# muhanzhang/IGMC

Measured on AMD Instinct MI355X. Metric: enclosing-subgraphs/sec (train step, batch=50) + test RMSE, higher is better.
Workload: dtype f32; 1 GPU; ml_1m, hop 1, max-nodes-per-hop 100, batch 50 per GPU, adj-dropout 0, dynamic-train, ARR 0.001, Adam; parallelism=dp1, global_batch=50, graphs_captured_before_timing=True, steps_per_graph_launch=100, group_steps=50

## Files before the change

igmc_amd/csrc/capi.hip:

```cpp
#include "launch.h"
#include "sortpool.h"
#include "g2_image.h"

#include <algorithm>
#include <climits>
#include <cmath>
#include <cstdio>
#include <cstring>
#include <map>
#include <string>
#include <vector>

static thread_local std::string g_err;
int g_igmc_prof_on = 0;

#define IGMC_FAIL(msg)                                                      \
  do {                                                                      \
    g_err = std::string(__func__) + ": " + (msg);                           \
    return 1;                                                               \
  } while (0)
#define HIPCHECK(expr)                                                      \
  do {                                                                      \
    hipError_t e_ = (expr);                                                 \
    if (e_ != hipSuccess) {                                                 \
// ... 652 lines not shown
    d.off_basis[l] = off; off += (int64_t)4 * fin * 32;
    d.off_root[l] = off;  off += (int64_t)fin * 32;
    d.off_bias[l] = off;  off += 32;
    d.off_att[l] = off;   off += (int64_t)d.R * 4;
  }
  d.off_l1w = off; off += (int64_t)128 * d.D;
  d.off_l1b = off; off += 128;
  d.off_l2w = off; off += 128;
  d.off_l2b = off; off += 1;
  d.n_params = off;
  d.node_cap = max_nodes;
  d.edge_cap = max_edges;
  d.graph_cap = max_graphs;
  Allocs& M = m->mem;
  int fail = 0;
  const size_t N = (size_t)max_nodes, Bc = (size_t)max_graphs;
  for (int l = 0; l < 4; ++l) fail |= M.get(&d.h[l], N * 32) | M.get(&d.dpre[l], N * 32);
  fail |= M.get(&d.agg, N * 128);
  for (int l = 0; l < 3; ++l) fail |= M.get(&d.gagg[l], N * 128) | M.get(&d.Y[l], N * 128);
  fail |= M.get(&d.feat, Bc * d.D) | M.get(&d.a1, Bc * 128) | M.get(&d.lmask, Bc * 128) | M.get(&d.dz, Bc * 128) |
          M.get(&d.gfeat, Bc * d.D) | M.get(&d.err, Bc) | M.get(&d.cnt0, N * d.R * d.L);
  const size_t rows0 = (size_t)d.R * d.L + d.L + 1;
  d.ts_part = nullptr;
  d.ts_raw = nullptr;
  d.ts_stride = (d.R * 32 + 33) * 32;
  d.fin_stash = nullptr;
  d.datt_part = nullptr;
  d.fold_w = nullptr;
  if (d.R <= G2_NR * G2_NG_MAX)
  {
    fail |= M.get(&d.ts_part, (size_t)4 * IGMC_TS_BLOCKS * d.ts_stride) |
            M.get(&d.ts_raw, (size_t)4 * d.ts_stride + (size_t)4 * d.ts_stride / 32 * 4);
    if (!fail) d.datt_part = d.ts_raw + (size_t)4 * d.ts_stride;
    fail |= M.get(&d.fold_w, (size_t)4 * 32 * IGMC_FOLD_NA);
  }
  if (d.R <= 128) fail |= M.get(&d.fin_stash, (size_t)4 * IGMC_STASH_LAYER + 16);
  d.g2_ex = nullptr;
  d.g2_fx = nullptr;
  d.g2_px = nullptr;
  d.g2_px_stride = 0;
  d.g2_w = nullptr;
  d.g2_graphs = 0;
  d.ex_nodes = 256;
  d.g2_ex_stride = (size_t)Bc * 2 * 32 * d.ex_nodes;
  const int wide = d.R <= G2_NR * G2_NG_MAX;
  const int xcd_ok = igmc_g2_xcd_ok();
  if (wide && Bc <= 2048 && xcd_ok) {
    fail |= M.get(&d.g2_ex, 5 * d.g2_ex_stride) | M.get(&d.g2_fx, Bc * 256) | M.get(&d.g2_w, g2_w_words(d.R, d.L));
    d.g2_graphs = (int)Bc;
    if (d.R <= G2_NR && Bc <= 1024) {
      d.g2_px_stride = (size_t)Bc * 2 * 32768;
      fail |= M.get(&d.g2_px, 5 * d.g2_px_stride);
    } else if (d.R <= G2_NR) {
      static bool told = false;
      if (!told) fprintf(stderr, "[igmc] batches of more than 1024 subgraphs: no plane-exchange regions -- the dense-layer / per-layer kernels take the steps, not the subgraph kernel\n");
      told = true;
    }
  } else if (wide) {
    fail |= M.get(&d.g2_w, g2_w_words(d.R, d.L));
  }
  fail |= M.get(&d.gs_bar, 2 * Bc + 1);
  fail |= M.get(&d.gs_ts, 4);
  d.gs_err = d.gs_bar ? d.gs_bar + 2 * Bc : nullptr;
  fail |= M.get(&d.wg_part, (size_t)4 * IGMC_WG_BLOCKS * igmc_wg_stride()) |
          M.get(&d.gatt_part, (size_t)3 * IGMC_GATHER_BLOCKS * d.R * 4) |
          M.get(&d.l0_part, (size_t)IGMC_L0_BLOCKS * rows0 * 32) |
          M.get(&d.graw, (size_t)3 * igmc_wg_stride() + 3 * d.R * 4 + rows0 * 32) | M.get(&d.arr_part, 4);
  d.side = nullptr;
  d.ctrl = nullptr;
  d.dcat[0] = d.dcat[1] = d.dcat[2] = nullptr;
  fail |= M.get(&m->done_ctr, 8);
  if (fail) {
    M.release();
    delete m;
    IGMC_FAIL("hipMalloc failed (model workspace)");
  }
  {
    hipStream_t st1, st2;
    if (hipStreamCreateWithFlags(&st1, hipStreamNonBlocking) != hipSuccess ||
        hipStreamCreateWithFlags(&st2, hipStreamNonBlocking) != hipSuccess) {
      M.release();
      delete m;
      IGMC_FAIL("hipStreamCreate failed");
    }
    m->ax.s1 = st1;
    m->ax.s2 = st2;
    for (int i = 0; i < 8; ++i) {
      hipEvent_t e;
      if (hipEventCreateWithFlags(&e, hipEventDisableTiming) != hipSuccess) IGMC_FAIL("hipEventCreate failed");
      m->ax.ev[i] = e;
    }
  }
  HIPCHECK(hipMemset(m->done_ctr, 0, 8 * sizeof(int)));
  HIPCHECK(hipMemset(m->d.gs_bar, 0, (2 * (size_t)max_graphs + 1) * sizeof(int)));
  {
    const unsigned long long ts0[4] = {~0ull, 0ull, 0ull, 0ull};
    HIPCHECK(hipMemcpy(m->d.gs_ts, ts0, sizeof(ts0), hipMemcpyHostToDevice));
  }
  if (m->d.fold_w) HIPCHECK(hipMemset(m->d.fold_w, 0, (size_t)4 * 32 * IGMC_FOLD_NA * sizeof(unsigned long long)));
  if (m->d.g2_ex) {
    HIPCHECK(hipMemset(m->d.g2_ex, 0, 5 * m->d.g2_ex_stride * sizeof(unsigned long long)));
    HIPCHECK(hipMemset(m->d.g2_fx, 0, (size_t)max_graphs * 256 * sizeof(unsigned long long)));
    if (m->d.g2_px) HIPCHECK(hipMemset(m->d.g2_px, 0, 5 * m->d.g2_px_stride));
  }
  if (igmc_model_prepare(d)) {
    M.release();
    delete m;
    IGMC_FAIL("hipFuncSetAttribute failed");
  }
  *out = m;
  return 0;
}

extern "C" int igmc_debug_lin_mask(const igmc_model* m, uint8_t* h_out, int64_t n) {
  if (!m || !h_out) IGMC_FAIL("null argument");
  if (n < 0 || n > (int64_t)m->d.graph_cap * 128) IGMC_FAIL("mask size out of range");
  HIPCHECK(hipDeviceSynchronize());
  HIPCHECK(hipMemcpy(h_out, m->d.lmask, (size_t)n, hipMemcpyDeviceToHost));
  return 0;
}

extern "C" int igmc_debug_head_array(const igmc_model* m, int which, float* h_out, int64_t n) {
  if (!m || !h_out) IGMC_FAIL("null argument");
  if (which < 0 || which > 3) IGMC_FAIL("no such array");
  const float* src = which == 0 ? m->d.a1 : which == 1 ? m->d.dz : which == 2 ? m->d.feat : m->d.gfeat;
  if (n < 0 || n > (int64_t)m->d.graph_cap * (which < 2 ? 128 : m->d.D)) IGMC_FAIL("size out of range");
  HIPCHECK(hipDeviceSynchronize());
  HIPCHECK(hipMemcpy(h_out, src, (size_t)n * sizeof(float), hipMemcpyDeviceToHost));
  return 0;
}

extern "C" int igmc_debug_weight_images(const igmc_model* m, float* h_out, int64_t* n_words) {
// ... 297 lines not shown

extern "C" int igmc_ctrl_tick(int64_t* d_ctrl, void* stream) {
  if (!d_ctrl) IGMC_FAIL("null ctrl");
  igmc_launch_tick(d_ctrl, stream);
  HIPCHECK(hipGetLastError());
  return 0;
}
extern "C" int igmc_ctrl_regroup(int64_t* d_ctrl, int M, int64_t first_cur, int64_t first_next, void* stream) {
  if (!d_ctrl || M < 1 || first_cur < 0 || first_next < 0) IGMC_FAIL("bad arguments");
  igmc_launch_regroup(d_ctrl, M, first_cur, first_next, stream);
  HIPCHECK(hipGetLastError());
  return 0;
}
extern "C" int igmc_ctrl_gate(int64_t* d_ctrl, int q, int gk_min, double delay_us, int delay_always, double timeout_us,
                              void* stream) {
  if (!d_ctrl || gk_min < 0 || !(timeout_us >= 0.0) || !(delay_us >= 0.0) || delay_us > 1000.0) IGMC_FAIL("bad arguments");
  igmc_launch_gate(d_ctrl, q & 1, gk_min, (long long)(delay_us * 100.0), delay_always != 0, (long long)(timeout_us * 100.0), stream);
  HIPCHECK(hipGetLastError());
  return 0;
}
extern "C" int igmc_batch_set_ctrl(igmc_batch* b, const int64_t* d_ctrl) {
  if (!b) IGMC_FAIL("null batch");
  b->ctrl = d_ctrl;
  return 0;
}
extern "C" int igmc_model_set_ctrl(igmc_model* m, const int64_t* d_ctrl) {
  if (!m) IGMC_FAIL("null model");
  m->d.ctrl = d_ctrl;
  return 0;
}
extern "C" int igmc_model_reset_exchange(igmc_model* m, void* stream) {
  if (!m) IGMC_FAIL("null model");
  hipStream_t st = (hipStream_t)stream;
  if (m->d.fold_w) HIPCHECK(hipMemsetAsync(m->d.fold_w, 0, (size_t)4 * 32 * IGMC_FOLD_NA * sizeof(unsigned long long), st));
  if (m->d.g2_ex) {
    HIPCHECK(hipMemsetAsync(m->d.g2_ex, 0, 5 * m->d.g2_ex_stride * sizeof(unsigned long long), st));
    HIPCHECK(hipMemsetAsync(m->d.g2_fx, 0, (size_t)m->d.g2_graphs * 256 * sizeof(unsigned long long), st));
    if (m->d.g2_px) HIPCHECK(hipMemsetAsync(m->d.g2_px, 0, 5 * m->d.g2_px_stride, st));
  }
  return 0;
}
extern "C" int igmc_model_check(igmc_model* m, void* stream) {
  if (!m) IGMC_FAIL("null model");
  int v = 0;
  if (m->d.gs_err) {
    HIPCHECK(hipStreamSynchronize((hipStream_t)stream));
    HIPCHECK(hipMemcpy(&v, m->d.gs_err, sizeof(int), hipMemcpyDeviceToHost));
    if (v) {
      HIPCHECK(hipMemset(m->d.gs_bar, 0, (2 * (size_t)m->d.graph_cap + 1) * sizeof(int)));
      (void)igmc_model_reset_exchange(m, stream);
      HIPCHECK(hipStreamSynchronize((hipStream_t)stream));
      IGMC_FAIL("a workgroup-cluster exchange of k_graph_step2 or a hand-off of the one-launch tail k_tail_fin timed out (GPU "
                "shared with another job?): results of the affected steps are invalid; set IGMC_GS_CLUSTER=1 or "
                "IGMC_GRAPH_STEP=0 (the tail alone: IGMC_TAIL_FOLD=0)");
    }
  }
  return 0;
}
extern "C" int igmc_adam_step_ctrl(float* d_params, const float* d_grad, float* d_exp_avg, float* d_exp_avg_sq,
                                   int64_t n, const int64_t* d_ctrl, void* stream) {
  if (!d_params || !d_grad || !d_exp_avg || !d_exp_avg_sq || n <= 0 || !d_ctrl) IGMC_FAIL("bad arguments");
  igmc_launch_adam(d_params, d_grad, d_exp_avg, d_exp_avg_sq, n, 0.f, 0.f, 0.f, 0.f, 0.f, 0.f, (int64_t*)d_ctrl, 0, stream);
  HIPCHECK(hipGetLastError());
  return 0;
}

extern "C" int igmc_step_finish(igmc_model* m, const igmc_batch* b, float* d_params, const float* d_grad,
// ... 604 lines not shown
```

igmc_amd/csrc/model.h:

```cpp
#pragma once
#include "common.h"

#define IGMC_KCAT 160
#ifndef IGMC_WG_BLOCKS
#define IGMC_WG_BLOCKS 64
#endif
#define IGMC_STASH_LAYER 672
#define IGMC_FOLD_NA 32
#define IGMC_TS_BLOCKS 256
#define IGMC_GATHER_BLOCKS 4096
#define IGMC_FBS_MAX_R 32
#define IGMC_L0_BLOCKS 256
#define IGMC_HG 8

struct ModelDev {
  int R, Bs, L, S, D;
  int64_t off_basis[4], off_root[4], off_bias[4], off_att[4];
  int64_t off_l1w, off_l1b, off_l2w, off_l2b, n_params;
  int node_cap, edge_cap, graph_cap;
  float* h[4];
  float* agg;
  float* gagg[3];
  float* Y[3];
  float* dpre[4];
  float* feat;
  float* a1;
  uint8_t* lmask;
  float* dz;
  float* gfeat;
  float* err;
  uint16_t* cnt0;
  float* wg_part;
  float* gatt_part;
  float* l0_part;
  float* graw;
  float* ts_part;
  float* ts_raw;
  int ts_stride;
  float* fin_stash;
  float* datt_part;
  unsigned long long* fold_w;
// ... 71 lines not shown
```

igmc_amd/csrc/model.hip:

```cpp
#include "model.h"
#include "g2_image.h"
#include "fin_stash.h"
#include "g2_words.h"
#include <stdlib.h>

struct XcdSeg {
  int lo, hi;
  int j, nj;
};
__device__ __forceinline__ XcdSeg igmc_xcd_segment(const BatchDev& b) {
  XcdSeg s;
  const int B = b.totals[3];
  const int x = blockIdx.x & 7;
  s.j = blockIdx.x >> 3;
  s.nj = (gridDim.x + 7 - x) >> 3;
  s.lo = b.node_off[(x * B) >> 3];
  s.hi = b.node_off[((x + 1) * B) >> 3];
  return s;
}


template <bool FLAGS, bool STORE>
__global__ __launch_bounds__(IGMC_BLOCK) void k_l0_fwd(BatchDev b, ModelDev m, const float* __restrict__ P,
                                                         float* __restrict__ out) {
  igmc_kernarg_warm<sizeof(BatchDev) + sizeof(ModelDev) + 32>();
  IGMC_DYN_SMEM(smem);
  const int RL = m.R * m.L, LF = m.L * 32;
  float* sW0 = (float*)smem;
  float* sroot = sW0 + RL * 32;
  float* sbias = sroot + LF;
  int* shist = (int*)(sbias + 32);
  for (int i = threadIdx.x; i < RL * 32; i += IGMC_BLOCK) {
    const int r = i / LF, cf = i % LF;
    float s = 0.f;
#pragma unroll
    for (int bb = 0; bb < 4; ++bb) s += P[m.off_att[0] + r * 4 + bb] * P[m.off_basis[0] + bb * LF + cf];
    sW0[i] = s;
// ... 1835 lines not shown
        const float anew = fts_att_entry(grad, at, st, R, rb, g, arr_coef, i, pold, m1o, m2o, part == 0);
        if (emit) s_attn[rb] = anew;
       }
      }
    }
    if (has) {
      if (table) {
        fts_col_table8(g, st, tv, R);
        for (int r = 8; r < R; ++r) {
          const float tvr = t0[(size_t)r * nE + e];
#pragma unroll
          for (int bb = 0; bb < 4; ++bb) g[bb] += st[IGMC_STASH_ATT + r * 4 + bb] * tvr;
        }
      }
      fts_col_emit(grad, at, st, arr_coef, idx, g, pv, m1v, m2v, pn);
      e_img = e;
    }
    if (emit) {
      __syncthreads();
      if (e_img >= 0) fts_image_col(m, ng, l, R, fin, e_img >> 5, e_img & 31, s_attn, pn, 0, 1);
    }
  } else if ((int)blockIdx.x < 4 * IGMC_FTS_NB + nlin) {
    const int64_t n_lin = m.n_params - m.off_l1w;
    const int64_t chunk = (n_lin + nlin - 1) / nlin;
    const int64_t lo = m.off_l1w + (int64_t)(blockIdx.x - 4 * IGMC_FTS_NB) * chunk;
    const int64_t hi = (lo + chunk < m.n_params) ? lo + chunk : m.n_params;
    adam_range<8>(at.p, grad, at.m1, at.m2, lo, hi, at.step_size, at.inv_sqrt_bc2, at.beta1, at.beta2, at.eps, at.wd);
  } else {
    loss_body(at.b, m, at.ARR, at.loss, at.total, smf);
    if (tid == 0 && at.ctrl) ctrl_check_and_advance(at.ctrl, at.b, at.use_flags);
  }
}

#define IGMC_TF_SETS 3
#define IGMC_TF_ROWS 384
#define IGMC_TF_O_ROWS (IGMC_TF_SETS * 1024)
#define IGMC_TF_O_ST (IGMC_TF_O_ROWS + IGMC_TF_ROWS)
#define IGMC_TF_O_DATT (IGMC_TF_O_ST + IGMC_STASH_LAYER)
#define IGMC_TF_O_ATTN (IGMC_TF_O_DATT + 32 * IGMC_FOLD_NA)
#define IGMC_TF_O_PN (IGMC_TF_O_ATTN + 64)
#define IGMC_TF_O_SMF (IGMC_TF_O_PN + 5 * 32)
#define IGMC_TF_WORDS (IGMC_TF_O_SMF + 16)
#define IGMC_TF_POLL ((32 * IGMC_FOLD_NA + IGMC_BLOCK - 1) / IGMC_BLOCK)
#define IGMC_TF_TIMEOUT_TICKS 20000000ll
#define IGMC_SYNC_ERR_FOLD 8

#if defined(IGMC_FIN_CLOCKS) && !defined(IGMC_HIPEMU)
__device__ unsigned long long g_fin_clk[64];
extern "C" int igmc_debug_fin_clocks(unsigned long long* out) {
  return hipMemcpyFromSymbol(out, HIP_SYMBOL(g_fin_clk), sizeof(g_fin_clk)) != hipSuccess;
}
#define TF_STAMP(on, k) do { if ((on) && threadIdx.x == 0) g_fin_clk[k] = __builtin_readcyclecounter(); } while (0)
#else
#define TF_STAMP(on, k) do { } while (0)
#endif

__global__ __launch_bounds__(IGMC_BLOCK) void k_tail_fin(BatchDev b, ModelDev m, const float* P, float grad_scale, float mult,
                                                           float drop_scale, float* grad, float arr_coef, AdamTail at, int nlin,
                                                           int nparts, int stride, int B, int bump_seq, int mute_layer) {
  __builtin_amdgcn_s_setprio(3);
  igmc_kernarg_warm<sizeof(BatchDev) + sizeof(ModelDev) + sizeof(AdamTail) + 64>();
  IGMC_DYN_SMEM(smem);
  float* S = (float*)smem;
  const int tid = threadIdx.x, lane = tid & 63, wave = tid >> 6;
  const float* stash = m.fin_stash;
  if (at.ctrl) {
    at.step_size = stash[IGMC_STASH_SCAL + 0];
    at.inv_sqrt_bc2 = stash[IGMC_STASH_SCAL + 1];
    at.beta1 = stash[IGMC_STASH_SCAL + 2];
    at.beta2 = stash[IGMC_STASH_SCAL + 3];
    at.eps = stash[IGMC_STASH_SCAL + 4];
    at.wd = stash[IGMC_STASH_SCAL + 5];
  }
  const int R = m.R, L = m.L, na = R * 4;
  const int nconv = 96 + L;
  const int blk = blockIdx.x;
  TF_STAMP(blk == 0, 0);
  TF_STAMP(blk == nconv, 16);
  TF_STAMP(blk == nconv + nlin, 32);
  if (blk < nconv) {
    const int l = blk < 96 ? 1 + (blk >> 5) : 0, c = blk < 96 ? (blk & 31) : blk - 96;
    const int fin = (l == 0) ? L : 32, nE = fin * 32, ts = m.ts_stride;
    const uint32_t tag = __float_as_uint(stash[IGMC_STASH_SCAL + IGMC_STASH_SEQ]) * 2u + 1u;
    float4* sred4 = (float4*)S;
    float* rows = S + IGMC_TF_O_ROWS;
    float* s_st = S + IGMC_TF_O_ST;
    float* s_datt = S + IGMC_TF_O_DATT;
    float* s_attn = S + IGMC_TF_O_ATTN;
    float* s_pn = S + IGMC_TF_O_PN;
    int* s_flag = (int*)(S + IGMC_TF_O_SMF + 8);
    const int ng = g2_groups(R, L);
    const int o4 = lane & 15, pg = wave * 4 + (lane >> 4);
    float stq[(IGMC_STASH_LAYER + IGMC_BLOCK - 1) / IGMC_BLOCK];
#pragma unroll
    for (int u = 0; u < (IGMC_STASH_LAYER + IGMC_BLOCK - 1) / IGMC_BLOCK; ++u) {
      const int i = tid + u * IGMC_BLOCK;
      stq[u] = stash[l * IGMC_STASH_LAYER + (i < IGMC_STASH_LAYER ? i : IGMC_STASH_LAYER - 1)];
    }
    const int f = tid & 31, e = c * 32 + f;
    const bool col = tid < 32, bias_role = c == 0 && tid >= 32 && tid < 64;
    int64_t idx[5];
    float pv[5], m1v[5], m2v[5], pvb[4] = {0.f, 0.f, 0.f, 0.f}, bq[4] = {0.f, 0.f, 0.f, 0.f};
#pragma unroll
    for (int q = 0; q < 5; ++q) {
      idx[q] = (q < 4) ? m.off_basis[l] + (int64_t)q * nE + e : m.off_root[l] + e;
      pv[q] = col ? P[idx[q]] : 0.f;
      m1v[q] = col ? at.m1[idx[q]] : 0.f;
      m2v[q] = col ? at.m2[idx[q]] : 0.f;
    }
    if (wave == 0) {
#pragma unroll
      for (int bb = 0; bb < 4; ++bb) pvb[bb] = P[idx[bb]];
    }
    if (bias_role) {
      const int64_t i = m.off_bias[l] + f;
      bq[1] = P[i];
      bq[2] = at.m1[i];
      bq[3] = at.m2[i];
    }
    if (tid == 0) *s_flag = 0;
    TF_STAMP(blk == 0, 1);
    const float* pl = m.ts_part + (size_t)l * IGMC_TS_BLOCKS * ts;
    const TsSlots sl = ts_slots(nparts, stride, B);
    const int nq = sl.nq;
    bool first_round = true;
    auto sum_columns = [&](int k0, int k1) {
      const int nsets = (k1 - k0 + 15) >> 4;
      int i0[IGMC_TF_SETS];
      float4 s4[IGMC_TF_SETS];
#pragma unroll
      for (int s = 0; s < IGMC_TF_SETS; ++s) {
        const int k = k0 + 16 * s + o4, kc = k < k1 ? k : k1 - 1, j = kc >> 3;
        const int row = j < R ? j * fin + c : j == R ? R * fin + c : R * fin + fin;
        i0[s] = row * 32 + 4 * (kc & 7);
        s4[s] = make_float4(0.f, 0.f, 0.f, 0.f);
      }
      for (int q0 = pg; q0 < nq; q0 += 16 * 14) {
        float4 v[IGMC_TF_SETS][14];
        size_t so[14];
#pragma unroll
        for (int u = 0; u < 14; ++u) so[u] = (size_t)ts_slot(sl, q0 + 16 * u) * ts;
#pragma unroll
        for (int s = 0; s < IGMC_TF_SETS; ++s)
          if (s < nsets) {
#pragma unroll
            for (int u = 0; u < 14; ++u) v[s][u] = *(const float4*)(pl + so[u] + i0[s]);
          }
#pragma unroll
        for (int s = 0; s < IGMC_TF_SETS; ++s)
          if (s < nsets) {
#pragma unroll
            for (int u = 0; u < 14; ++u)
              if (q0 + 16 * u < nq) {
                s4[s].x += v[s][u].x; s4[s].y += v[s][u].y; s4[s].z += v[s][u].z; s4[s].w += v[s][u].w;
              }
          }
      }
      if (!first_round) __syncthreads();
#pragma unroll
      for (int s = 0; s < IGMC_TF_SETS; ++s)
        if (s < nsets) sred4[(s * 16 + pg) * 16 + o4] = s4[s];
      if (first_round) {
#pragma unroll
        for (int u = 0; u < (IGMC_STASH_LAYER + IGMC_BLOCK - 1) / IGMC_BLOCK; ++u) {
          const int i = tid + u * IGMC_BLOCK;
          if (i < IGMC_STASH_LAYER) s_st[i] = stq[u];
        }
      }
      first_round = false;
      __syncthreads();
      if (wave < nsets) {
        const float* sr = (const float*)sred4;
        float tot = 0.f;
#pragma unroll
        for (int g16 = 0; g16 < 16; ++g16) tot += sr[((wave * 16 + g16) * 16 + (lane >> 2)) * 4 + (lane & 3)];
        const int k = k0 + 16 * wave + (lane >> 2);
        if (k < k1) rows[k * 4 + (lane & 3)] = tot;
      }
    };
    const int ncol_a = 8 * (R + 1);
    for (int k0 = 0; k0 < ncol_a; k0 += 16 * IGMC_TF_SETS) sum_columns(k0, k0 + 16 * IGMC_TF_SETS < ncol_a ? k0 + 16 * IGMC_TF_SETS : ncol_a);
    __syncthreads();
    TF_STAMP(blk == 0, 2);
    unsigned long long* words = m.fold_w + (size_t)l * 32 * IGMC_FOLD_NA;
    if (wave == 0) {
      const int h = lane >> 5;
      for (int r2 = 0; r2 < R; r2 += 2) {
        const int r = r2 + h;
        const float tot = r < R ? rows[r * 32 + f] : 0.f;
        float pb[4];
#pragma unroll
        for (int bb = 0; bb < 4; ++bb) pb[bb] = tot * pvb[bb];
#pragma unroll
        for (int bb = 0; bb < 4; ++bb)
#pragma unroll
          for (int d = 16; d >= 1; d >>= 1) pb[bb] += __shfl_xor(pb[bb], d, 64);
#ifdef IGMC_HIPEMU
        if (l == mute_layer) continue;
#endif
        if (f == 0 && r < R) {
#pragma unroll
          for (int bb = 0; bb < 4; ++bb) g2_pub_f32_agent(words + c * IGMC_FOLD_NA + r * 4 + bb, pb[bb], tag);
        }
      }
    }
    TF_STAMP(blk == 0, 3);
    if (c == 0) sum_columns(ncol_a, ncol_a + 8);
    TF_STAMP(blk == 0, 4);
    {
      const int nw = fin * na;
      const unsigned long long* wp[IGMC_TF_POLL];
      int wi[IGMC_TF_POLL];
#pragma unroll
      for (int u = 0; u < IGMC_TF_POLL; ++u) {
        const int w = tid + u * IGMC_BLOCK, wc = w < nw ? w : nw - 1;
        wi[u] = (wc / na) * IGMC_FOLD_NA + wc % na;
        wp[u] = words + wi[u];
      }
      bool ok = false;
#ifndef IGMC_HIPEMU
      const long long t0 = (long long)wall_clock64();
#endif
      for (long it = 0;; ++it) {
        unsigned long long w[IGMC_TF_POLL];
        bool all = true;
#pragma unroll
        for (int u = 0; u < IGMC_TF_POLL; ++u) w[u] = g2_ld_word(wp[u]);
#pragma unroll
        for (int u = 0; u < IGMC_TF_POLL; ++u) all = all && (uint32_t)(w[u] >> 32) == tag;
        if (all) {
#pragma unroll
          for (int u = 0; u < IGMC_TF_POLL; ++u) s_datt[wi[u]] = __uint_as_float((uint32_t)w[u]);
          ok = true;
          break;
        }
#ifndef IGMC_HIPEMU
        if ((it & 15) == 15 && (long long)wall_clock64() - t0 > IGMC_TF_TIMEOUT_TICKS) break;
        __builtin_amdgcn_s_sleep(2);
#else
        if (it > (1L << 12)) break;
        hipemu::yield();
#endif
      }
      if (!ok) *s_flag = 1;
    }
    __syncthreads();
    TF_STAMP(blk == 0, 5);
    if (*s_flag) {
      if (tid == 0) {
        *m.gs_err = 1;
        if (at.ctrl) atomicOr((unsigned long long*)(at.ctrl + IGMC_CTRL_SYNC_ERR), (unsigned long long)IGMC_SYNC_ERR_FOLD);
      }
      return;
    }
    const float* st = s_st;
    if (tid >= 64 && tid - 64 < na) {
      const int rb = tid - 64;
      float g = 0.f;
#pragma unroll
      for (int k = 0; k < 32; ++k) g += (k < fin) ? s_datt[k * IGMC_FOLD_NA + rb] : 0.f;
      s_attn[rb] = fts_att_entry(grad, at, st, R, rb, g, arr_coef, m.off_att[l] + rb, st[IGMC_STASH_ATT + rb],
                                 st[IGMC_STASH_ATTM1 + rb], st[IGMC_STASH_ATTM2 + rb], c == 0);
    }
    if (bias_role) {
      bq[0] = rows[(R + 1) * 32 + f];
      fts_bias(m, grad, at, ng, l, R, fin, f, bq, true);
    }
    if (col) {
      float g[5] = {0.f, 0.f, 0.f, 0.f, 0.f}, tv[8], pn[5];
#pragma unroll
      for (int r = 0; r < 8; ++r) tv[r] = (r < R) ? rows[r * 32 + f] : 0.f;
      g[4] = rows[R * 32 + f];
      fts_col_table8(g, st, tv, R);
      fts_col_emit(grad, at, st, arr_coef, idx, g, pv, m1v, m2v, pn);
#pragma unroll
      for (int q = 0; q < 5; ++q) s_pn[q * 32 + f] = pn[q];
    }
    TF_STAMP(blk == 0, 6);
    __syncthreads();
    {
      float pn[5];
#pragma unroll
      for (int q = 0; q < 5; ++q) pn[q] = s_pn[q * 32 + f];
      fts_image_col(m, ng, l, R, fin, c, f, s_attn, pn, tid >> 5, IGMC_BLOCK / 32);
    }
    TF_STAMP(blk == 0, 7);
  } else if (blk < nconv + nlin) {
    const int bx = (blk - nconv) & 7, by = (blk - nconv) >> 3, D = m.D;
    head_bwd_w_body(b, m, P, nullptr, 1, grad_scale, mult, drop_scale, grad, bx, by, B);
    __syncthreads();
    TF_STAMP(blk == nconv, 17);
    int64_t ix[5];
    bool okx[5];
    float gv[5], pv[5], av[5], vv[5];
#pragma unroll
    for (int k = 0; k < 4; ++k) {
      const int el = tid + k * IGMC_BLOCK, colx = by * 64 + (el & 63);
      okx[k] = colx < D;
      ix[k] = m.off_l1w + (int64_t)(bx * 16 + (el >> 6)) * D + (okx[k] ? colx : 0);
    }
    okx[4] = by == 0 && (tid < 32 || (tid == 32 && bx == 0));
    ix[4] = tid < 16 ? m.off_l1b + bx * 16 + tid : tid < 32 ? m.off_l2w + bx * 16 + tid - 16 : m.off_l2b;
    const float* gsrc = grad;
#pragma unroll
    for (int k = 0; k < 5; ++k) {
      const int64_t i = okx[k] ? ix[k] : m.off_l1w;
      gv[k] = gsrc[i];
      pv[k] = at.p[i];
      av[k] = at.m1[i];
      vv[k] = at.m2[i];
    }
#pragma unroll
    for (int k = 0; k < 5; ++k)
      if (okx[k]) adam_store_sep(at.p, at.m1, at.m2, ix[k], gv[k], pv[k], av[k], vv[k], at.step_size, at.inv_sqrt_bc2, at.beta1,
                                 at.beta2, at.eps, at.wd);
    TF_STAMP(blk == nconv, 18);
  } else {
    if (bump_seq && tid == 0) m.gs_bar[1] += 1;
    loss_body(at.b, m, at.ARR, at.loss, at.total, S + IGMC_TF_O_SMF);
    TF_STAMP(true, 33);
    if (tid == 0 && at.ctrl) ctrl_check_and_advance(at.ctrl, at.b, at.use_flags);
    TF_STAMP(true, 34);
  }
}

__global__ __launch_bounds__(IGMC_BLOCK) void k_loss(BatchDev b, ModelDev m, float ARR, float* __restrict__ loss) {
  igmc_kernarg_warm<sizeof(BatchDev) + sizeof(ModelDev) + 32>();
  __shared__ float smf[8];
  loss_body(b, m, ARR, loss, nullptr, smf);
}

__global__ __launch_bounds__(IGMC_BLOCK) void k_sse_acc(BatchDev b, const float* __restrict__ out, double* acc, int64_t* ctrl) {
  igmc_kernarg_warm<sizeof(BatchDev) + 32>();
  __shared__ float smf[8];
  const int B = b.totals[3];
  float s = 0.f;
  for (int g = threadIdx.x; g < B; g += IGMC_BLOCK) {
    const float d = out[g] - b.y[g];
    s += d * d;
  }
  s = igmc_block_sum_f(s, smf);
  if (threadIdx.x == 0) {
    acc[0] += (double)s;
    acc[1] += (double)B;
    if (ctrl) ctrl_advance(ctrl);
  }
}

__global__ void k_tick(int64_t* ctrl) {
// ... 121 lines not shown
                              int tables, void* stream) {
  const int gt = igmc_xcd_grid(m, B, 16, 2048);
  const size_t bsm4 = (size_t)(16 * IGMC_TP + 1024 + m.R * 4 + 16 * m.R * 4) * sizeof(float);
  for (int l = 3; l >= 1; --l) {
    if (sp.bwd_dense) igmc_launch_dl_layer(m, b, P, B, l, 1, use_flags, nullptr, stream, tables);
    else igmc_dispatch([&](auto uf) {
      IGMC_PLAUNCH("k_rgcn_layer_bwd", (k_rgcn_layer4<uf(), true>), gt, IGMC_BLOCK, bsm4, stream, b, m, P, l, (float*)nullptr);
    }, use_flags != 0);
  }
}

static void launch_reduce(const ModelDev& m, const BatchDev& b, const StepPlan& sp, const float* P, int B, const int64_t* ctrl,
                          int nstash, void* stream) {
  const int rows0 = m.R * m.L + m.L + 1, l0_mfma = rows0 <= 32;
  const float* d0 = m.dpre[0];
  if (l0_mfma) {
  } else if (rows0 <= 64) IGMC_PLAUNCH("k_l0_bwd", (k_l0_bwd<8>), IGMC_L0_BLOCKS, IGMC_BLOCK, 0, stream, b, m, d0, m.l0_part);
  else IGMC_PLAUNCH("k_l0_bwd", (k_l0_bwd<40>), IGMC_L0_BLOCKS, IGMC_BLOCK, 0, stream, b, m, d0, m.l0_part);
  const int nblk = ((l0_mfma ? 4 : 3) * igmc_wg_stride() + 63) / 64 + (l0_mfma ? 0 : (rows0 * 32 + 63) / 64) + (3 * m.R * 4 + 3) / 4;
  IGMC_PLAUNCH("k_reduce_partials", k_reduce_partials, nblk + nstash, IGMC_BLOCK, 0, stream, m,
               sp.bwd_dense ? sp.dl_grid : igmc_xcd_grid(m, B, 16, 2048), l0_mfma, IGMC_WG_BLOCKS, P, ctrl, nstash);
}

static void launch_tail_ts(const ModelDev& m, const BatchDev& b, const float* P, int B, float grad_scale, float mult, float* grad,
                           int nlin, int nparts, int stride, int nstash, const int64_t* ctrl, int bump_seq, void* stream) {
  IGMC_PLAUNCH("k_tail_ts", k_tail_ts, nlin + (4 * m.ts_stride + 63) / 64 + nstash, IGMC_BLOCK, 0, stream, b, m, P, grad_scale,
               mult, 2.f, grad, nlin, nparts, stride, B, nstash, ctrl, bump_seq);
}

static void launch_tail_fin(const ModelDev& m, const BatchDev& b, const float* P, int B, float grad_scale, float mult, float* grad,
                            float arr_coef, const AdamTail& at, int nlin, int nparts, int stride, int bump_seq, void* stream) {
  int mute = -1;
#ifdef IGMC_HIPEMU
  if (const char* e = getenv("IGMC_EMU_FOLD_MUTE")) mute = atoi(e);
  hipemu::rt().co_cs = 32;
  hipemu::rt().co_stride = -1;
  hipemu::rt().co_block = 0;
#endif
  IGMC_PLAUNCH("k_tail_fin", k_tail_fin, 96 + m.L + nlin + 1, IGMC_BLOCK, (size_t)IGMC_TF_WORDS * sizeof(float), stream, b, m, P,
               grad_scale, mult, 2.f, grad, arr_coef, at, nlin, nparts, stride, B, bump_seq, mute);
}

static int launch_exchange(const ModelDev& m, int tail, const StepExchange* xch, float* grad, void* stream) {
  if (!xch || tail == IGMC_TAIL_HANDOFF) return 0;
  const int rows0 = m.R * m.L + m.L + 1;
  const int64_t n = tail == IGMC_TAIL_TS ? (int64_t)4 * m.ts_stride + (int64_t)4 * m.ts_stride / 32 * 4
                                         : (int64_t)3 * igmc_wg_stride() + 3 * m.R * 4 + rows0 * 32;
  return xch->sum(xch->user, tail == IGMC_TAIL_TS ? m.ts_raw : m.graw, n, grad + m.off_l1w, m.n_params - m.off_l1w, stream);
}

static void launch_finalize(const ModelDev& m, const BatchDev& b, const float* P, float* grad, float arr_coef, int tail,
                            int ts_mode, const AdamTail& at, int img, float ARR, float* loss, int* img_emitted, void* stream) {
  const int bs = tail == IGMC_TAIL_BS;
  if (tail == IGMC_TAIL_HANDOFF) {
    if (at.enabled) IGMC_PLAUNCH("k_finalize_adam", k_finalize, 4 * IGMC_FIN_NB + 32, IGMC_BLOCK, 0, stream, m, P, grad, arr_coef, at, ts_mode);
    else IGMC_PLAUNCH("k_finalize", k_finalize, 4 * IGMC_FIN_NB, IGMC_BLOCK, 0, stream, m, P, grad, arr_coef, at, ts_mode);
  } else if (at.enabled) {
    IGMC_PLAUNCH("k_finalize_adam", k_finalize_ts, 4 * IGMC_FTS_NB + 32 + 1, IGMC_BLOCK, 0, stream, m, P, grad, arr_coef, at, 32, bs, img);
    if (img_emitted) *img_emitted = img;
  } else {
    IGMC_PLAUNCH("k_finalize", k_finalize_ts, 4 * IGMC_FTS_NB, IGMC_BLOCK, 0, stream, m, P, grad, arr_coef, at, 0, bs, 0);
  }
  if (!at.enabled && loss) igmc_launch_loss(m, b, ARR, loss, stream);
}


void igmc_launch_forward(const ModelDev& m, const BatchDev& b, const StepPlan& sp, const float* P, int B, int training,
                         int use_flags, const uint8_t* inj_mask, uint64_t seed, uint64_t step, float mult,
                         float* out, void* stream) {
  if (sp.family == IGMC_FAM_G2) {
    igmc_launch_graph_step2(m, b, sp, P, B, 0, use_flags, nullptr, seed, step, mult, 0.f, out, stream);
    return;
// ... 203 lines not shown
```

igmc_amd/stepgraph.py:

```python
import ctypes as C
import os
import struct
import sys

import numpy as np
import torch

from . import _lib, parallel

MAX_GROUP = 50
SPARSE_CANDIDATES = 128.0
GROUP_EXTRACT_CHUNK = 2


def _ctrl_words(step, epoch, adam_t, batch, group, lr, beta1, beta2, eps, wd):
    w = np.zeros(_lib.CTRL['WORDS'], dtype=np.int64)
    w[_lib.CTRL['STEP']], w[_lib.CTRL['EPOCH']], w[_lib.CTRL['K']] = step, epoch, 0
    w[_lib.CTRL['FIRST']], w[_lib.CTRL['FIRST_ODD']] = 0, group * batch
    w[_lib.CTRL['GROUP']], w[_lib.CTRL['GK']], w[_lib.CTRL['GQ']] = group, 0, 0
    w[_lib.CTRL['ADAM_T']], w[_lib.CTRL['BATCH']] = adam_t, batch
    step_size = float(lr) / (1.0 - float(beta1) ** adam_t)
    inv_sqrt_bc2 = 1.0 / (1.0 - float(beta2) ** adam_t) ** 0.5
    for key, val in (('LR', lr), ('BETA1', beta1), ('BETA2', beta2), ('EPS', eps), ('WD', wd),
                     ('STEP_SIZE', step_size), ('INV_SQRT_BC2', inv_sqrt_bc2)):
        w[_lib.CTRL[key]] = struct.unpack('<q', struct.pack('<d', float(val)))[0]
    return w


def _group_size(steps_hint, default):
    n = int(steps_hint)
    if 4 <= n <= MAX_GROUP:
        return n
    for m in range(MAX_GROUP, 3, -1):
# ... 484 lines not shown
        if self.sp is not None:
            self._sortpool_step(arena, B)
        elif self.dp_path and os.environ.get('IGMC_DP_FLAT', '0') != '1':
            self._train_step_dp(arena)
        elif not self.dp_path and B == self.B:
            self._train_step(arena)
        else:
            self._model(arena, B)
            self._finish(arena)

    @property
    def graphs(self):
        return [self.graph] + list(self.graph1)

    def drop_graphs(self):
        self.graph, self.graph1 = None, [None, None]

    def _capture(self):
        if self.graph is not None or not self.use_graph:
            return self.graph
        self.graph = self._capture_fn(self._enqueue_pair)
        return self.graph

    def _capture_single(self, q):
        if self.graph1[q] is not None or not self.use_graph:
            return self.graph1[q]
        self.graph1[q] = self._capture_fn(lambda: self._enqueue_group(q, standalone=True))
        return self.graph1[q]

    def _capture_fn(self, enqueue):
        for qq in (0, 1):
            self._arena(qq, self.M - 1)
            self._batch_sets(qq)
        torch.cuda.synchronize()
        g = torch.cuda.CUDAGraph()
        dist = parallel.is_dist()
        try:
            with torch.cuda.graph(g, **(dict(capture_error_mode='thread_local') if dist else {})):
                enqueue()
        except RuntimeError as e:
            if self.comm is None and not dist:
                raise
            sys.stderr.write('igmc_amd: hipGraph capture refused under data parallelism (%s); launching eagerly\n'
                             % str(e).splitlines()[0])
            self.use_graph, self.graph, self.graph1, g = False, None, [None, None], None
            torch.cuda.synchronize()
        if self.comm is not None:
            parallel.barrier()
        return g

    def prepare(self, steps_hint=None, group=None, prime=True):
        if not self.use_graph or self.steps_done < 1 or not self._attached:
            return False
        M = self.M
        if group is not None:
            M = max(1, min(MAX_GROUP, int(group)))
        elif steps_hint:
            M = _group_size(steps_hint, self.M_default)
        if M != self.M:
            self.M = M
            self.drop_graphs()
            self.avail = 0
        if self.gq != 0 or self.gk != 0 or self.avail < self.M:
            self._regroup()
        single = steps_hint is not None and self.M <= int(steps_hint) < 2 * self.M
        self.single_launch = bool(single)
        have = (lambda: self.graph1[0] if self.graph1[1] is not None else None) if single else (lambda: self.graph)
        cap = (lambda: (self._capture_single(0), self._capture_single(1))) if single else self._capture
        order = (lambda: [self.graph1[0], self.graph1[1], self.graph1[0]]) if single else (lambda: [self.graph] * 3)
        fresh = have() is None
        cap()
        if fresh and have() is not None and prime and self.avail >= self.M and \
                self.n_links // self.B - self.k >= 2 * self.M:
            self._prime(order())
            if have() is None and self.use_graph:
                cap()
                if have() is not None:
                    self._prime(order())
        return self.use_graph
# ... 139 lines not shown
```

Before: 825,700 subgraphs/s.

## Split tail column reductions across producer blocks with cross-block word exchange

Inside k_tail_fin, the per-layer column-set reductions over ts_part were done serially by each conv block. They are now spread across extra producer blocks, one per column set (plus bias-row blocks). Each producer publishes its sums and its datt contributions through tagged fold_w words, and the conv blocks poll for those words. The aim is to shorten the tail's critical path by raising parallelism, at the cost of more blocks, extra exchange memory and more polling traffic. Python GC is also disabled during graph capture.

```diff
diff --git a/igmc_amd/csrc/capi.hip b/igmc_amd/csrc/capi.hip
--- a/igmc_amd/csrc/capi.hip
+++ b/igmc_amd/csrc/capi.hip
@@ -708,7 +708,7 @@
     fail |= M.get(&d.ts_part, (size_t)4 * IGMC_TS_BLOCKS * d.ts_stride) |
             M.get(&d.ts_raw, (size_t)4 * d.ts_stride + (size_t)4 * d.ts_stride / 32 * 4);
     if (!fail) d.datt_part = d.ts_raw + (size_t)4 * d.ts_stride;
-    fail |= M.get(&d.fold_w, (size_t)4 * 32 * IGMC_FOLD_NA);
+    fail |= M.get(&d.fold_w, (size_t)IGMC_FOLD_WORDS);
   }
   if (d.R <= 128) fail |= M.get(&d.fin_stash, (size_t)4 * IGMC_STASH_LAYER + 16);
   d.g2_ex = nullptr;
@@ -773,7 +773,7 @@
     const unsigned long long ts0[4] = {~0ull, 0ull, 0ull, 0ull};
     HIPCHECK(hipMemcpy(m->d.gs_ts, ts0, sizeof(ts0), hipMemcpyHostToDevice));
   }
-  if (m->d.fold_w) HIPCHECK(hipMemset(m->d.fold_w, 0, (size_t)4 * 32 * IGMC_FOLD_NA * sizeof(unsigned long long)));
+  if (m->d.fold_w) HIPCHECK(hipMemset(m->d.fold_w, 0, (size_t)IGMC_FOLD_WORDS * sizeof(unsigned long long)));
   if (m->d.g2_ex) {
     HIPCHECK(hipMemset(m->d.g2_ex, 0, 5 * m->d.g2_ex_stride * sizeof(unsigned long long)));
     HIPCHECK(hipMemset(m->d.g2_fx, 0, (size_t)max_graphs * 256 * sizeof(unsigned long long)));
@@ -1137,7 +1137,7 @@
 extern "C" int igmc_model_reset_exchange(igmc_model* m, void* stream) {
   if (!m) IGMC_FAIL("null model");
   hipStream_t st = (hipStream_t)stream;
-  if (m->d.fold_w) HIPCHECK(hipMemsetAsync(m->d.fold_w, 0, (size_t)4 * 32 * IGMC_FOLD_NA * sizeof(unsigned long long), st));
+  if (m->d.fold_w) HIPCHECK(hipMemsetAsync(m->d.fold_w, 0, (size_t)IGMC_FOLD_WORDS * sizeof(unsigned long long), st));
   if (m->d.g2_ex) {
     HIPCHECK(hipMemsetAsync(m->d.g2_ex, 0, 5 * m->d.g2_ex_stride * sizeof(unsigned long long), st));
     HIPCHECK(hipMemsetAsync(m->d.g2_fx, 0, (size_t)m->d.g2_graphs * 256 * sizeof(unsigned long long), st));
diff --git a/igmc_amd/csrc/model.h b/igmc_amd/csrc/model.h
--- a/igmc_amd/csrc/model.h
+++ b/igmc_amd/csrc/model.h
@@ -7,6 +7,10 @@
 #endif
 #define IGMC_STASH_LAYER 672
 #define IGMC_FOLD_NA 32
+#define IGMC_FOLD_PSETS 4
+#define IGMC_FOLD_O_ROWS (4 * 32 * IGMC_FOLD_NA)
+#define IGMC_FOLD_O_BIAS (IGMC_FOLD_O_ROWS + 4 * 32 * IGMC_FOLD_PSETS * 64)
+#define IGMC_FOLD_WORDS (IGMC_FOLD_O_BIAS + 4 * 32)
 #define IGMC_TS_BLOCKS 256
 #define IGMC_GATHER_BLOCKS 4096
 #define IGMC_FBS_MAX_R 32
diff --git a/igmc_amd/csrc/model.hip b/igmc_amd/csrc/model.hip
--- a/igmc_amd/csrc/model.hip
+++ b/igmc_amd/csrc/model.hip
@@ -3,6 +3,7 @@
 #include "fin_stash.h"
 #include "g2_words.h"
 #include <stdlib.h>
+#include <string.h>
 
 struct XcdSeg {
   int lo, hi;
@@ -1904,16 +1905,15 @@
   }
 }
 
-#define IGMC_TF_SETS 3
 #define IGMC_TF_ROWS 384
-#define IGMC_TF_O_ROWS (IGMC_TF_SETS * 1024)
+#define IGMC_TF_O_ROWS 1024
 #define IGMC_TF_O_ST (IGMC_TF_O_ROWS + IGMC_TF_ROWS)
 #define IGMC_TF_O_DATT (IGMC_TF_O_ST + IGMC_STASH_LAYER)
 #define IGMC_TF_O_ATTN (IGMC_TF_O_DATT + 32 * IGMC_FOLD_NA)
 #define IGMC_TF_O_PN (IGMC_TF_O_ATTN + 64)
 #define IGMC_TF_O_SMF (IGMC_TF_O_PN + 5 * 32)
 #define IGMC_TF_WORDS (IGMC_TF_O_SMF + 16)
-#define IGMC_TF_POLL ((32 * IGMC_FOLD_NA + IGMC_BLOCK - 1) / IGMC_BLOCK)
+#define IGMC_TF_POLL ((IGMC_FOLD_PSETS * 64 + 32 * IGMC_FOLD_NA + 32 + IGMC_BLOCK - 1) / IGMC_BLOCK)
 #define IGMC_TF_TIMEOUT_TICKS 20000000ll
 #define IGMC_SYNC_ERR_FOLD 8
 
@@ -1927,15 +1927,108 @@
 #define TF_STAMP(on, k) do { } while (0)
 #endif
 
+__device__ __forceinline__ float tf_sum_set(const float* __restrict__ pl, const TsSlots& sl, int ts, int R, int fin, int c,
+                                            int k0, int k1, float4* sred4) {
+  const int lane = threadIdx.x & 63, wave = threadIdx.x >> 6;
+  const int o4 = lane & 15, pg = wave * 4 + (lane >> 4);
+  const int k = k0 + o4, kc = k < k1 ? k : k1 - 1, j = kc >> 3;
+  const int row = j < R ? j * fin + c : j == R ? R * fin + c : R * fin + fin;
+  const int i0 = row * 32 + 4 * (kc & 7);
+  float4 s4 = make_float4(0.f, 0.f, 0.f, 0.f);
+  const int nq = sl.nq;
+  for (int q0 = pg; q0 < nq; q0 += 16 * 14) {
+    float4 v[14];
+#pragma unroll
+    for (int u = 0; u < 14; ++u) v[u] = *(const float4*)(pl + (size_t)ts_slot(sl, q0 + 16 * u) * ts + i0);
+#pragma unroll
+    for (int u = 0; u < 14; ++u)
+      if (q0 + 16 * u < nq) {
+        s4.x += v[u].x; s4.y += v[u].y; s4.z += v[u].z; s4.w += v[u].w;
+      }
+  }
+  sred4[pg * 16 + o4] = s4;
+  __syncthreads();
+  float tot = 0.f;
+  if (wave == 0) {
+    const float* sr = (const float*)sred4;
+#pragma unroll
+    for (int g16 = 0; g16 < 16; ++g16) tot += sr[(g16 * 16 + (lane >> 2)) * 4 + (lane & 3)];
+  }
+  return tot;
+}
+
+__device__ __forceinline__ void tf_datt_pub(float tot, int r, int R, const float (&pvb)[4], unsigned long long* wrow, uint32_t tag,
+                                            bool mute) {
+  const int f = threadIdx.x & 31;
+  if (r >= R) tot = 0.f;
+  float pb[4];
+#pragma unroll
+  for (int bb = 0; bb < 4; ++bb) pb[bb] = tot * pvb[bb];
+#pragma unroll
+  for (int bb = 0; bb < 4; ++bb)
+#pragma unroll
+    for (int d = 16; d >= 1; d >>= 1) pb[bb] += __shfl_xor(pb[bb], d, 64);
+  if (mute) return;
+  if (f == 0 && r < R) {
+#pragma unroll
+    for (int bb = 0; bb < 4; ++bb) g2_pub_f32_agent(wrow + r * 4 + bb, pb[bb], tag);
+  }
+}
+
 __global__ __launch_bounds__(IGMC_BLOCK) void k_tail_fin(BatchDev b, ModelDev m, const float* P, float grad_scale, float mult,
                                                            float drop_scale, float* grad, float arr_coef, AdamTail at, int nlin,
-                                                           int nparts, int stride, int B, int bump_seq, int mute_layer) {
+                                                           int nparts, int stride, int B, int bump_seq, int mute) {
   __builtin_amdgcn_s_setprio(3);
   igmc_kernarg_warm<sizeof(BatchDev) + sizeof(ModelDev) + sizeof(AdamTail) + 64>();
   IGMC_DYN_SMEM(smem);
   float* S = (float*)smem;
   const int tid = threadIdx.x, lane = tid & 63, wave = tid >> 6;
   const float* stash = m.fin_stash;
+  const int R = m.R, L = m.L, na = R * 4;
+  const int nconv = 96 + L;
+  const int ncol_a = 8 * (R + 1), nsets = (ncol_a + 15) >> 4;
+  const int nprod_r = (nsets - 1) * nconv, nprod = (nprod_r + 4 + 31) & ~31;
+  const int blk = blockIdx.x;
+#ifdef IGMC_HIPEMU
+  const int mute_layer = mute < 0 ? -1 : (mute & 255), mute_role = mute < 0 ? 0 : (mute >> 8);
+#else
+  const int mute_layer = -1, mute_role = 0;
+#endif
+  TF_STAMP(blk == nprod, 0);
+  TF_STAMP(blk == nprod + nconv, 16);
+  TF_STAMP(blk == nprod + nconv + nlin, 32);
+  TF_STAMP(blk == 0, 40);
+  TF_STAMP(blk == nprod_r + 1, 48);
+  if (blk < nprod) {
+    if (blk >= nprod_r + 4) return;
+    const bool brow = blk >= nprod_r;
+    const int mi = brow ? 0 : blk / (nsets - 1), set = brow ? 0 : 1 + blk % (nsets - 1);
+    const int l = brow ? blk - nprod_r : mi < 96 ? 1 + (mi >> 5) : 0, c = brow ? 0 : mi < 96 ? (mi & 31) : mi - 96;
+    const int fin = (l == 0) ? L : 32, nE = fin * 32, ts = m.ts_stride;
+    const uint32_t tag = __float_as_uint(stash[IGMC_STASH_SCAL + IGMC_STASH_SEQ]) * 2u + 1u;
+    float pvb[4] = {0.f, 0.f, 0.f, 0.f};
+    if (wave == 0 && !brow) {
+#pragma unroll
+      for (int bb = 0; bb < 4; ++bb) pvb[bb] = P[m.off_basis[l] + (int64_t)bb * nE + c * 32 + (lane & 31)];
+    }
+    TF_STAMP(blk == 0, 41);
+    TF_STAMP(blk == nprod_r + 1, 49);
+    const TsSlots sl = ts_slots(nparts, stride, B);
+    const int k0 = brow ? ncol_a : 16 * set, k1 = brow ? ncol_a + 8 : (k0 + 16 < ncol_a ? k0 + 16 : ncol_a);
+    const float tot = tf_sum_set(m.ts_part + (size_t)l * IGMC_TS_BLOCKS * ts, sl, ts, R, fin, c, k0, k1, (float4*)S);
+    TF_STAMP(blk == 0, 42);
+    TF_STAMP(blk == nprod_r + 1, 50);
+    if (wave == 0) {
+      const bool silent = l == mute_layer && mute_role != (brow ? 1 : 2);
+      unsigned long long* w = brow ? m.fold_w + IGMC_FOLD_O_BIAS + l * 32
+                                   : m.fold_w + IGMC_FOLD_O_ROWS + (size_t)((l * 32 + c) * IGMC_FOLD_PSETS + set - 1) * 64;
+      if (!silent && k0 + (lane >> 2) < k1) g2_pub_f32_agent(w + lane, tot, tag);
+      if (!brow) tf_datt_pub(tot, 2 * set + (lane >> 5), R, pvb, m.fold_w + (size_t)(l * 32 + c) * IGMC_FOLD_NA, tag, silent);
+    }
+    TF_STAMP(blk == 0, 43);
+    TF_STAMP(blk == nprod_r + 1, 51);
+    return;
+  }
   if (at.ctrl) {
     at.step_size = stash[IGMC_STASH_SCAL + 0];
     at.inv_sqrt_bc2 = stash[IGMC_STASH_SCAL + 1];
@@ -1944,14 +2037,9 @@
     at.eps = stash[IGMC_STASH_SCAL + 4];
     at.wd = stash[IGMC_STASH_SCAL + 5];
   }
-  const int R = m.R, L = m.L, na = R * 4;
-  const int nconv = 96 + L;
-  const int blk = blockIdx.x;
-  TF_STAMP(blk == 0, 0);
-  TF_STAMP(blk == nconv, 16);
-  TF_STAMP(blk == nconv + nlin, 32);
-  if (blk < nconv) {
-    const int l = blk < 96 ? 1 + (blk >> 5) : 0, c = blk < 96 ? (blk & 31) : blk - 96;
+  const int mb = blk - nprod;
+  if (mb < nconv) {
+    const int l = mb < 96 ? 1 + (mb >> 5) : 0, c = mb < 96 ? (mb & 31) : mb - 96;
     const int fin = (l == 0) ? L : 32, nE = fin * 32, ts = m.ts_stride;
     const uint32_t tag = __float_as_uint(stash[IGMC_STASH_SCAL + IGMC_STASH_SEQ]) * 2u + 1u;
     float4* sred4 = (float4*)S;
@@ -1962,7 +2050,6 @@
     float* s_pn = S + IGMC_TF_O_PN;
     int* s_flag = (int*)(S + IGMC_TF_O_SMF + 8);
     const int ng = g2_groups(R, L);
-    const int o4 = lane & 15, pg = wave * 4 + (lane >> 4);
     float stq[(IGMC_STASH_LAYER + IGMC_BLOCK - 1) / IGMC_BLOCK];
 #pragma unroll
     for (int u = 0; u < (IGMC_STASH_LAYER + IGMC_BLOCK - 1) / IGMC_BLOCK; ++u) {
@@ -1991,103 +2078,39 @@
       bq[3] = at.m2[i];
     }
     if (tid == 0) *s_flag = 0;
-    TF_STAMP(blk == 0, 1);
-    const float* pl = m.ts_part + (size_t)l * IGMC_TS_BLOCKS * ts;
+    TF_STAMP(mb == 0, 1);
     const TsSlots sl = ts_slots(nparts, stride, B);
-    const int nq = sl.nq;
-    bool first_round = true;
-    auto sum_columns = [&](int k0, int k1) {
-      const int nsets = (k1 - k0 + 15) >> 4;
-      int i0[IGMC_TF_SETS];
-      float4 s4[IGMC_TF_SETS];
-#pragma unroll
-      for (int s = 0; s < IGMC_TF_SETS; ++s) {
-        const int k = k0 + 16 * s + o4, kc = k < k1 ? k : k1 - 1, j = kc >> 3;
-        const int row = j < R ? j * fin + c : j == R ? R * fin + c : R * fin + fin;
-        i0[s] = row * 32 + 4 * (kc & 7);
-        s4[s] = make_float4(0.f, 0.f, 0.f, 0.f);
-      }
-      for (int q0 = pg; q0 < nq; q0 += 16 * 14) {
-        float4 v[IGMC_TF_SETS][14];
-        size_t so[14];
-#pragma unroll
-        for (int u = 0; u < 14; ++u) so[u] = (size_t)ts_slot(sl, q0 + 16 * u) * ts;
-#pragma unroll
-        for (int s = 0; s < IGMC_TF_SETS; ++s)
-          if (s < nsets) {
-#pragma unroll
-            for (int u = 0; u < 14; ++u) v[s][u] = *(const float4*)(pl + so[u] + i0[s]);
-          }
-#pragma unroll
-        for (int s = 0; s < IGMC_TF_SETS; ++s)
-          if (s < nsets) {
-#pragma unroll
-            for (int u = 0; u < 14; ++u)
-              if (q0 + 16 * u < nq) {
-                s4[s].x += v[s][u].x; s4[s].y += v[s][u].y; s4[s].z += v[s][u].z; s4[s].w += v[s][u].w;
-              }
-          }
-      }
-      if (!first_round) __syncthreads();
-#pragma unroll
-      for (int s = 0; s < IGMC_TF_SETS; ++s)
-        if (s < nsets) sred4[(s * 16 + pg) * 16 + o4] = s4[s];
-      if (first_round) {
-#pragma unroll
-        for (int u = 0; u < (IGMC_STASH_LAYER + IGMC_BLOCK - 1) / IGMC_BLOCK; ++u) {
-          const int i = tid + u * IGMC_BLOCK;
-          if (i < IGMC_STASH_LAYER) s_st[i] = stq[u];
-        }
-      }
-      first_round = false;
-      __syncthreads();
-      if (wave < nsets) {
-        const float* sr = (const float*)sred4;
-        float tot = 0.f;
-#pragma unroll
-        for (int g16 = 0; g16 < 16; ++g16) tot += sr[((wave * 16 + g16) * 16 + (lane >> 2)) * 4 + (lane & 3)];
-        const int k = k0 + 16 * wave + (lane >> 2);
-        if (k < k1) rows[k * 4 + (lane & 3)] = tot;
-      }
-    };
-    const int ncol_a = 8 * (R + 1);
-    for (int k0 = 0; k0 < ncol_a; k0 += 16 * IGMC_TF_SETS) sum_columns(k0, k0 + 16 * IGMC_TF_SETS < ncol_a ? k0 + 16 * IGMC_TF_SETS : ncol_a);
-    __syncthreads();
-    TF_STAMP(blk == 0, 2);
+#pragma unroll
+    for (int u = 0; u < (IGMC_STASH_LAYER + IGMC_BLOCK - 1) / IGMC_BLOCK; ++u) {
+      const int i = tid + u * IGMC_BLOCK;
+      if (i < IGMC_STASH_LAYER) s_st[i] = stq[u];
+    }
+    const float tot = tf_sum_set(m.ts_part + (size_t)l * IGMC_TS_BLOCKS * ts, sl, ts, R, fin, c, 0, ncol_a < 16 ? ncol_a : 16, sred4);
+    if (wave == 0 && (lane >> 2) < ncol_a) rows[lane] = tot;
+    TF_STAMP(mb == 0, 2);
     unsigned long long* words = m.fold_w + (size_t)l * 32 * IGMC_FOLD_NA;
-    if (wave == 0) {
-      const int h = lane >> 5;
-      for (int r2 = 0; r2 < R; r2 += 2) {
-        const int r = r2 + h;
-        const float tot = r < R ? rows[r * 32 + f] : 0.f;
-        float pb[4];
-#pragma unroll
-        for (int bb = 0; bb < 4; ++bb) pb[bb] = tot * pvb[bb];
-#pragma unroll
-        for (int bb = 0; bb < 4; ++bb)
-#pragma unroll
-          for (int d = 16; d >= 1; d >>= 1) pb[bb] += __shfl_xor(pb[bb], d, 64);
-#ifdef IGMC_HIPEMU
-        if (l == mute_layer) continue;
-#endif
-        if (f == 0 && r < R) {
-#pragma unroll
-          for (int bb = 0; bb < 4; ++bb) g2_pub_f32_agent(words + c * IGMC_FOLD_NA + r * 4 + bb, pb[bb], tag);
-        }
-      }
-    }
-    TF_STAMP(blk == 0, 3);
-    if (c == 0) sum_columns(ncol_a, ncol_a + 8);
-    TF_STAMP(blk == 0, 4);
+    if (wave == 0) tf_datt_pub(tot, lane >> 5, R, pvb, words + c * IGMC_FOLD_NA, tag, l == mute_layer && mute_role == 0);
+    TF_STAMP(mb == 0, 3);
     {
-      const int nw = fin * na;
+      const int nrw = 4 * ncol_a - 64, ndw = fin * na, nw = nrw + ndw + 32, npoll = (nw + IGMC_BLOCK - 1) / IGMC_BLOCK;
+      const unsigned long long* wrow = m.fold_w + IGMC_FOLD_O_ROWS + (size_t)(l * 32 + c) * IGMC_FOLD_PSETS * 64;
       const unsigned long long* wp[IGMC_TF_POLL];
       int wi[IGMC_TF_POLL];
 #pragma unroll
       for (int u = 0; u < IGMC_TF_POLL; ++u) {
         const int w = tid + u * IGMC_BLOCK, wc = w < nw ? w : nw - 1;
-        wi[u] = (wc / na) * IGMC_FOLD_NA + wc % na;
-        wp[u] = words + wi[u];
+        if (wc < nrw) {
+          wp[u] = wrow + wc;
+          wi[u] = IGMC_TF_O_ROWS + 64 + wc;
+        } else if (wc < nrw + ndw) {
+          const int x = wc - nrw, y = (x / na) * IGMC_FOLD_NA + x % na;
+          wp[u] = words + y;
+          wi[u] = IGMC_TF_O_DATT + y;
+        } else {
+          const int x = wc - nrw - ndw;
+          wp[u] = m.fold_w + IGMC_FOLD_O_BIAS + l * 32 + x;
+          wi[u] = IGMC_TF_O_ROWS + (R + 1) * 32 + x;
+        }
       }
       bool ok = false;
 #ifndef IGMC_HIPEMU
@@ -2097,12 +2120,14 @@
         unsigned long long w[IGMC_TF_POLL];
         bool all = true;
 #pragma unroll
-        for (int u = 0; u < IGMC_TF_POLL; ++u) w[u] = g2_ld_word(wp[u]);
-#pragma unroll
-        for (int u = 0; u < IGMC_TF_POLL; ++u) all = all && (uint32_t)(w[u] >> 32) == tag;
+        for (int u = 0; u < IGMC_TF_POLL; ++u)
+          if (u < npoll) w[u] = g2_ld_word(wp[u]);
+#pragma unroll
+        for (int u = 0; u < IGMC_TF_POLL; ++u) all = all && (u >= npoll || (uint32_t)(w[u] >> 32) == tag);
         if (all) {
 #pragma unroll
-          for (int u = 0; u < IGMC_TF_POLL; ++u) s_datt[wi[u]] = __uint_as_float((uint32_t)w[u]);
+          for (int u = 0; u < IGMC_TF_POLL; ++u)
+            if (u < npoll) S[wi[u]] = __uint_as_float((uint32_t)w[u]);
           ok = true;
           break;
         }
@@ -2117,7 +2142,7 @@
       if (!ok) *s_flag = 1;
     }
     __syncthreads();
-    TF_STAMP(blk == 0, 5);
+    TF_STAMP(mb == 0, 5);
     if (*s_flag) {
       if (tid == 0) {
         *m.gs_err = 1;
@@ -2148,7 +2173,7 @@
 #pragma unroll
       for (int q = 0; q < 5; ++q) s_pn[q * 32 + f] = pn[q];
     }
-    TF_STAMP(blk == 0, 6);
+    TF_STAMP(mb == 0, 6);
     __syncthreads();
     {
       float pn[5];
@@ -2156,12 +2181,12 @@
       for (int q = 0; q < 5; ++q) pn[q] = s_pn[q * 32 + f];
       fts_image_col(m, ng, l, R, fin, c, f, s_attn, pn, tid >> 5, IGMC_BLOCK / 32);
     }
-    TF_STAMP(blk == 0, 7);
-  } else if (blk < nconv + nlin) {
-    const int bx = (blk - nconv) & 7, by = (blk - nconv) >> 3, D = m.D;
+    TF_STAMP(mb == 0, 7);
+  } else if (mb < nconv + nlin) {
+    const int bx = (mb - nconv) & 7, by = (mb - nconv) >> 3, D = m.D;
     head_bwd_w_body(b, m, P, nullptr, 1, grad_scale, mult, drop_scale, grad, bx, by, B);
     __syncthreads();
-    TF_STAMP(blk == nconv, 17);
+    TF_STAMP(mb == nconv, 17);
     int64_t ix[5];
     bool okx[5];
     float gv[5], pv[5], av[5], vv[5];
@@ -2186,7 +2211,7 @@
     for (int k = 0; k < 5; ++k)
       if (okx[k]) adam_store_sep(at.p, at.m1, at.m2, ix[k], gv[k], pv[k], av[k], vv[k], at.step_size, at.inv_sqrt_bc2, at.beta1,
                                  at.beta2, at.eps, at.wd);
-    TF_STAMP(blk == nconv, 18);
+    TF_STAMP(mb == nconv, 18);
   } else {
     if (bump_seq && tid == 0) m.gs_bar[1] += 1;
     loss_body(at.b, m, at.ARR, at.loss, at.total, S + IGMC_TF_O_SMF);
@@ -2374,12 +2399,17 @@
                             float arr_coef, const AdamTail& at, int nlin, int nparts, int stride, int bump_seq, void* stream) {
   int mute = -1;
 #ifdef IGMC_HIPEMU
-  if (const char* e = getenv("IGMC_EMU_FOLD_MUTE")) mute = atoi(e);
+  if (const char* e = getenv("IGMC_EMU_FOLD_MUTE")) {
+    mute = atoi(e);
+    const char* role = getenv("IGMC_EMU_FOLD_MUTE_ROLE");
+    if (mute >= 0 && role) mute |= (!strcmp(role, "rows") ? 1 : !strcmp(role, "bias") ? 2 : 0) << 8;
+  }
   hipemu::rt().co_cs = 32;
   hipemu::rt().co_stride = -1;
   hipemu::rt().co_block = 0;
 #endif
-  IGMC_PLAUNCH("k_tail_fin", k_tail_fin, 96 + m.L + nlin + 1, IGMC_BLOCK, (size_t)IGMC_TF_WORDS * sizeof(float), stream, b, m, P,
+  const int nconv = 96 + m.L, nsets = (8 * (m.R + 1) + 15) / 16, nprod = ((nsets - 1) * nconv + 4 + 31) & ~31;
+  IGMC_PLAUNCH("k_tail_fin", k_tail_fin, nprod + nconv + nlin + 1, IGMC_BLOCK, (size_t)IGMC_TF_WORDS * sizeof(float), stream, b, m, P,
                grad_scale, mult, 2.f, grad, arr_coef, at, nlin, nparts, stride, B, bump_seq, mute);
 }
 
diff --git a/igmc_amd/stepgraph.py b/igmc_amd/stepgraph.py
--- a/igmc_amd/stepgraph.py
+++ b/igmc_amd/stepgraph.py
@@ -1,4 +1,5 @@
 import ctypes as C
+import gc
 import os
 import struct
 import sys
@@ -549,6 +550,9 @@
         for qq in (0, 1):
             self._arena(qq, self.M - 1)
             self._batch_sets(qq)
+        gc.collect()
+        gc_on = gc.isenabled()
+        gc.disable()
         torch.cuda.synchronize()
         g = torch.cuda.CUDAGraph()
         dist = parallel.is_dist()
@@ -562,6 +566,9 @@
                              % str(e).splitlines()[0])
             self.use_graph, self.graph, self.graph1, g = False, None, [None, None], None
             torch.cuda.synchronize()
+        finally:
+            if gc_on:
+                gc.enable()
         if self.comm is not None:
             parallel.barrier()
         return g
```

Measured after the change: 841,800 subgraphs/s (median of 6 runs). 1.02x the previous value.
